# wkvong/multimodal-baby

Measured on AMD Instinct MI355X. Metric: image-text pairs/sec, CVCL ResNeXt+embed 224², bs256, 1/2/4/8 MI355X, higher is better.
Workload: dtype bf16; 1 GPU; C2 = BASELINE configs[1]: CVCL saycam_contrastive, frozen random-init ResNeXt-50 32x4d (BN train mode) + embedding mean-pool text encoder, E=512, L2-normalised, fixed tau 0.07, 224x224 frames + 3-word utterances; full step = fwd + InfoNCE + bwd(fc, embedding) + AdamW; per_gpu_batch=256, global_batch=256, negatives=local (single GPU), parallelism=dp1, trunk_streams=2

## Files before the change

### multimodal-baby_amd/csrc/gemm_pro.hip

```cpp
#include <cstdlib>

#include "cvcl_common.h"

namespace {

constexpr int PM = 64;
constexpr int PN = 256;

struct ProDev {
    const bf16_t* A; const bf16_t* W; bf16_t* C; const bf16_t* R;
    const float* a_scale; const float* a_shift; const float* c_scale; const float* c_shift; const float* r_scale; const float* r_shift;
    float* stats;
    int stats_acc;
    const float* centre;
    int M, N, lda, ldw, ldc, ldr;
    int tiles;
    const bf16_t* A2; const bf16_t* W2; const float* centre2;
    int lda2, ldw2;
};

enum { PRO_STATS = 0, PRO_STORE = 1, PRO_TAIL = 2, PRO_TAIL_DS = 3 };
constexpr int K2 = 64, KT2 = 2;
constexpr int X2BUF = PM * K2 * 2;

template <int KT> constexpr int pro_lds_bytes() { return 2 * PM * KT * 64 + 8 * 4096 + 6 * PN * 4 + 2 * 256 * 4 + 2 * X2BUF; }

template <int KT, int MODE, int D>
__global__ __launch_bounds__(512, 2) void gemm_pro_kernel(ProDev p) {
    constexpr bool TAIL = MODE == PRO_TAIL || MODE == PRO_TAIL_DS, DS = MODE == PRO_TAIL_DS;
    constexpr int K = KT * 32;
    constexpr int PITCH = K * 2;
    constexpr int CPR = K / 8;
    constexpr int NCH = PM * CPR / 512;
    constexpr int RPP = 512 / CPR;
    constexpr int ABUF = PM * PITCH;
    extern __shared__ __attribute__((aligned(16))) char smem[];
    const int tid = threadIdx.x, lane = tid & 63;
    const int wave = __builtin_amdgcn_readfirstlane(tid >> 6);
    const int wm = wave >> 2, wn = wave & 3;
    const int n0 = blockIdx.y * PN;

    bf16x8 fw[4][KT];
#pragma unroll
    for (int ni = 0; ni < 4; ++ni)
#pragma unroll
        for (int ks = 0; ks < KT; ++ks)
            fw[ni][ks] = *reinterpret_cast<const bf16x8*>(p.W + (long)(n0 + wn * 64 + ni * 16 + (lane & 15)) * p.ldw + ks * 32 + (lane >> 4) * 8);

    const int s_c = tid % CPR, s_r = tid / CPR;
    constexpr bool AFF_LDS = KT == 8;
    float* in_aff = reinterpret_cast<float*>(smem + 2 * ABUF + 8 * 4096 + 6 * PN * 4);
    char* x2buf = smem + 2 * ABUF + 8 * 4096 + 6 * PN * 4 + 2 * 256 * 4;
    const bool plain = p.a_scale == nullptr;
    const short fl = plain ? (short)-32768 : (short)0;
    const s16x2 floor2 = s16x2{fl, fl};
    f32x2 sc[4], sh[4];
#pragma unroll
    for (int e = 0; e < 4; ++e) { sc[e] = f32x2{1.f, 1.f}; sh[e] = f32x2{0.f, 0.f}; }
    if constexpr (AFF_LDS) {
        if (tid < K) { in_aff[tid] = plain ? 1.f : p.a_scale[tid]; in_aff[K + tid] = plain ? 0.f : p.a_shift[tid]; }
        __syncthreads();
    } else if (!plain) {
#pragma unroll
        for (int e = 0; e < 4; ++e) {
            sc[e] = f32x2{p.a_scale[s_c * 8 + 2 * e], p.a_scale[s_c * 8 + 2 * e + 1]};
            sh[e] = f32x2{p.a_shift[s_c * 8 + 2 * e], p.a_shift[s_c * 8 + 2 * e + 1]};
        }
    }
    u32x4 araw[D][NCH];
    auto load_a = [&](int tile, int slot) __attribute__((always_inline)) {
#pragma unroll
        for (int i = 0; i < NCH; ++i) {
            int m = tile * PM + s_r + RPP * i;
            if (m >= p.M) m = p.M - 1;
            araw[slot][i] = *reinterpret_cast<const u32x4*>(p.A + (long)m * p.lda + s_c * 8);
        }
    };
    auto stage_a = [&](int buf, int slot) __attribute__((always_inline)) {
        char* dst = smem + buf * ABUF;
        if constexpr (AFF_LDS) {
#pragma unroll
            for (int e = 0; e < 4; ++e) {
                sc[e] = *reinterpret_cast<const f32x2*>(in_aff + s_c * 8 + 2 * e);
                sh[e] = *reinterpret_cast<const f32x2*>(in_aff + K + s_c * 8 + 2 * e);
            }
        }
#pragma unroll
        for (int i = 0; i < NCH; ++i) {
            const int r = s_r + RPP * i;
            u32x4 v;
#pragma unroll
            for (int e = 0; e < 4; ++e) {
                const unsigned y = round2(__builtin_elementwise_fma(widen2(araw[slot][i][e]), sc[e], sh[e]));
                v[e] = __builtin_bit_cast(unsigned, __builtin_elementwise_max(__builtin_bit_cast(s16x2, y), floor2));
            }
            *reinterpret_cast<u32x4*>(dst + r * PITCH + ((s_c ^ (r & 15)) << 4)) = v;
        }
    };
    const int f_row = lane & 15, f_kc = lane >> 4;

    const int r_chunk = lane & 7, r_row0 = lane >> 3;
    float* aff = reinterpret_cast<float*>(smem + 2 * ABUF + 8 * 4096);
    if (tid < PN) aff[4 * PN + tid] = p.centre ? -p.centre[n0 + tid] : 0.f;
    if constexpr (DS) { if (tid < PN) aff[5 * PN + tid] = p.centre2 ? -p.centre2[n0 + tid] : 0.f; }
    const float* cen = aff + 4 * PN + wn * 64 + (lane >> 4) * 4;
    bf16x8 fw2[DS ? 4 : 1][DS ? KT2 : 1];
    u32x4 x2raw[DS ? D : 1];
    const int x_r = tid >> 3, x_c = tid & 7;
    if constexpr (DS) {
#pragma unroll
        for (int ni = 0; ni < 4; ++ni)
#pragma unroll
            for (int ks = 0; ks < KT2; ++ks)
                fw2[ni][ks] = *reinterpret_cast<const bf16x8*>(p.W2 + (long)(n0 + wn * 64 + ni * 16 + (lane & 15)) * p.ldw2 + ks * 32 + (lane >> 4) * 8);
    }
    auto load_x2 = [&](int tile, int slot) __attribute__((always_inline)) {
        int m = tile * PM + x_r;
        if (m >= p.M) m = p.M - 1;
        x2raw[slot] = *reinterpret_cast<const u32x4*>(p.A2 + (long)m * p.lda2 + x_c * 8);
    };
    auto stage_x2 = [&](int buf, int slot) __attribute__((always_inline)) {
        *reinterpret_cast<u32x4*>(x2buf + buf * X2BUF + x_r * 128 + ((x_c ^ (x_r & 7)) << 4)) = x2raw[slot];
    };
    if constexpr (TAIL) {
        if (tid < PN) {
            aff[tid] = p.c_scale[n0 + tid];
            aff[PN + tid] = p.c_shift[n0 + tid];
            aff[2 * PN + tid] = p.r_scale ? p.r_scale[n0 + tid] : 1.f;
            aff[3 * PN + tid] = p.r_scale ? p.r_shift[n0 + tid] : 0.f;
        }
    }
    bf16x8 rres[4];
    auto load_r = [&](int tile) __attribute__((always_inline)) {
#pragma unroll
        for (int j = 0; j < 4; ++j) {
            int m = tile * PM + wm * 32 + j * 8 + r_row0;
            if (m >= p.M) m = p.M - 1;
            rres[j] = *reinterpret_cast<const bf16x8*>(p.R + (long)m * p.ldr + n0 + wn * 64 + r_chunk * 8);
        }
    };
    f32x2 st_sum[8], st_sq[8];
#pragma unroll
    for (int e = 0; e < 8; ++e) { st_sum[e] = f32x2{0.f, 0.f}; st_sq[e] = f32x2{0.f, 0.f}; }

    char* stg = smem + 2 * ABUF + wave * 4096;
    const int e_row = lane & 15, e_wchunk = lane >> 5, e_wsub = ((lane >> 4) & 1) * 8;

    const int first = blockIdx.x;
    const int G = gridDim.x;
#pragma unroll
    for (int d = 0; d < D; ++d)
        if (first + d * G < p.tiles) {
            load_a(first + d * G, d);
            if constexpr (DS) load_x2(first + d * G, d);
        }
    if constexpr (MODE == PRO_TAIL) {
        if (first < p.tiles) load_r(first);
    }
    f32x4 acc[4][2];
    auto tile_stats = [&](int m0) __attribute__((always_inline)) {
#pragma unroll
        for (int mi = 0; mi < 2; ++mi) {
            const unsigned keep = m0 + mi * 16 + e_row < p.M ? 0xffffffffu : 0u;
#pragma unroll
            for (int ni = 0; ni < 4; ++ni)
#pragma unroll
                for (int h = 0; h < 2; ++h) {
                    const f32x2 f = widen2(round2(f32x2{acc[ni][mi][2 * h], acc[ni][mi][2 * h + 1]}) & keep);
                    st_sum[ni * 2 + h] += f;
                    st_sq[ni * 2 + h] = __builtin_elementwise_fma(f, f, st_sq[ni * 2 + h]);
                }
        }
    };
    int buf = 0;
    for (int tile = first; tile < p.tiles;) {
#pragma unroll
      for (int slot = 0; slot < D; ++slot) {
        if (tile >= p.tiles) break;
        stage_a(buf, slot);
        if constexpr (DS) stage_x2(buf, slot);
        __syncthreads();
        const int next = tile + G;
        if (tile + D * G < p.tiles) {
            load_a(tile + D * G, slot);
            if constexpr (DS) load_x2(tile + D * G, slot);
        }
        unsigned r2[DS ? 4 : 1][2][2];
        if constexpr (DS) {
            f32x4 acc2[4][2];
            const float* cen2 = aff + 5 * PN + wn * 64 + (lane >> 4) * 4;
#pragma unroll
            for (int ni = 0; ni < 4; ++ni) {
                const f32x4 c4 = *reinterpret_cast<const f32x4*>(cen2 + ni * 16);
#pragma unroll
                for (int mi = 0; mi < 2; ++mi) acc2[ni][mi] = c4;
            }
            const char* xb = x2buf + buf * X2BUF + (wm * 32 + f_row) * 128;
#pragma unroll
            for (int ks = 0; ks < KT2; ++ks) {
                bf16x8 fx[2];
#pragma unroll
                for (int mi = 0; mi < 2; ++mi)
                    fx[mi] = *reinterpret_cast<const bf16x8*>(xb + mi * 16 * 128 + (((ks * 4 + f_kc) ^ (f_row & 7)) << 4));
#pragma unroll
                for (int ni = 0; ni < 4; ++ni)
#pragma unroll
                    for (int mi = 0; mi < 2; ++mi)
                        acc2[ni][mi] = __builtin_amdgcn_mfma_f32_16x16x32_bf16(fw2[ni][ks], fx[mi], acc2[ni][mi], 0, 0, 0);
            }
#pragma unroll
            for (int ni = 0; ni < 4; ++ni)
#pragma unroll
                for (int mi = 0; mi < 2; ++mi) {
                    r2[ni][mi][0] = round2(f32x2{acc2[ni][mi][0], acc2[ni][mi][1]});
                    r2[ni][mi][1] = round2(f32x2{acc2[ni][mi][2], acc2[ni][mi][3]});
                }
        }
#pragma unroll
        for (int ni = 0; ni < 4; ++ni) {
            const f32x4 c4 = *reinterpret_cast<const f32x4*>(cen + ni * 16);
#pragma unroll
            for (int mi = 0; mi < 2; ++mi) acc[ni][mi] = c4;
        }
        const char* ab = smem + buf * ABUF + (wm * 32 + f_row) * PITCH;
#pragma unroll
        for (int ks = 0; ks < KT; ++ks) {
            bf16x8 fa[2];
#pragma unroll
            for (int mi = 0; mi < 2; ++mi)
                fa[mi] = *reinterpret_cast<const bf16x8*>(ab + mi * 16 * PITCH + (((ks * 4 + f_kc) ^ f_row) << 4));
#pragma unroll
            for (int ni = 0; ni < 4; ++ni)
#pragma unroll
                for (int mi = 0; mi < 2; ++mi)
                    acc[ni][mi] = __builtin_amdgcn_mfma_f32_16x16x32_bf16(fw[ni][ks], fa[mi], acc[ni][mi], 0, 0, 0);
        }
        const int m0 = tile * PM + wm * 32;
        if constexpr (MODE == PRO_STATS) {
            tile_stats(m0);
        } else if constexpr (DS) {
#pragma unroll
            for (int ni = 0; ni < 4; ++ni) {
                const float* t = aff + wn * 64 + ni * 16 + (lane >> 4) * 4;
                const f32x4 cs = *reinterpret_cast<const f32x4*>(t), cb = *reinterpret_cast<const f32x4*>(t + PN);
                const f32x4 rs = *reinterpret_cast<const f32x4*>(t + 2 * PN), rb = *reinterpret_cast<const f32x4*>(t + 3 * PN);
#pragma unroll
                for (int mi = 0; mi < 2; ++mi) {
                    bf16x4 q;
#pragma unroll
                    for (int e = 0; e < 4; ++e) {
                        const float y = fmaf((float)(bf16_t)acc[ni][mi][e], cs[e], cb[e]);
                        const float idv = fmaf(widen2(r2[ni][mi][e >> 1])[e & 1], rs[e], rb[e]);
                        q[e] = (bf16_t)fmaxf(y + idv, 0.f);
                    }
                    const int row = mi * 16 + e_row, chunk = ni * 2 + e_wchunk;
                    *reinterpret_cast<bf16x4*>(stg + row * 128 + ((chunk ^ ((row >> 1) & 7)) << 4) + e_wsub) = q;
                }
            }
#pragma unroll
            for (int j = 0; j < 4; ++j) {
                const int row = j * 8 + r_row0;
                const bf16x8 v = *reinterpret_cast<const bf16x8*>(stg + row * 128 + ((r_chunk ^ ((row >> 1) & 7)) << 4));
                const int m = m0 + row, n = n0 + wn * 64 + r_chunk * 8;
                if (m < p.M) stream_store(v, reinterpret_cast<bf16x8*>(p.C + (long)m * p.ldc + n));
            }
        } else {
#pragma unroll
            for (int mi = 0; mi < 2; ++mi)
#pragma unroll
                for (int ni = 0; ni < 4; ++ni) {
                    const bf16x4 q = {(bf16_t)acc[ni][mi][0], (bf16_t)acc[ni][mi][1], (bf16_t)acc[ni][mi][2], (bf16_t)acc[ni][mi][3]};
                    const int row = mi * 16 + e_row, chunk = ni * 2 + e_wchunk;
                    *reinterpret_cast<bf16x4*>(stg + row * 128 + ((chunk ^ ((row >> 1) & 7)) << 4) + e_wsub) = q;
                }
            float cs[8], cb[8], rs[8], rb[8];
            if constexpr (MODE == PRO_TAIL) {
                const float* t = aff + wn * 64 + r_chunk * 8;
#pragma unroll
                for (int e = 0; e < 8; ++e) { cs[e] = t[e]; cb[e] = t[PN + e]; rs[e] = t[2 * PN + e]; rb[e] = t[3 * PN + e]; }
            }
#pragma unroll
            for (int j = 0; j < 4; ++j) {
                const int row = j * 8 + r_row0;
                bf16x8 v = *reinterpret_cast<const bf16x8*>(stg + row * 128 + ((r_chunk ^ ((row >> 1) & 7)) << 4));
                const int m = m0 + row, n = n0 + wn * 64 + r_chunk * 8;
                if (m < p.M) {
                    if constexpr (MODE == PRO_TAIL) {
                        const bf16x8 r = rres[j];
#pragma unroll
                        for (int e = 0; e < 8; ++e) {
                            const float y = fmaf((float)v[e], cs[e], cb[e]);
                            const float idv = fmaf((float)r[e], rs[e], rb[e]);
                            v[e] = (bf16_t)fmaxf(y + idv, 0.f);
                        }
                    } else {
                        const u32x4 u = __builtin_bit_cast(u32x4, v);
#pragma unroll
                        for (int e = 0; e < 4; ++e) {
                            const f32x2 f = widen2(u[e]);
                            st_sum[e] += f;
                            st_sq[e] = __builtin_elementwise_fma(f, f, st_sq[e]);
                        }
                    }
                    stream_store(v, reinterpret_cast<bf16x8*>(p.C + (long)m * p.ldc + n));
                }
            }
            if constexpr (MODE == PRO_TAIL) {
                if (next < p.tiles) load_r(next);
            }
        }
        buf ^= 1;
        tile += G;
      }
    }

    if (!TAIL && p.stats) {
        __syncthreads();
        float* red = (float*)smem;
        if constexpr (MODE == PRO_STATS) {
#pragma unroll
            for (int e = 0; e < 8; ++e)
#pragma unroll
                for (int h = 0; h < 2; ++h)
#pragma unroll
                    for (int o = 1; o < 16; o <<= 1) {
                        st_sum[e][h] += __shfl_xor(st_sum[e][h], o, 64);
                        st_sq[e][h] += __shfl_xor(st_sq[e][h], o, 64);
                    }
            if ((lane & 15) == 0) {
#pragma unroll
                for (int ni = 0; ni < 4; ++ni)
#pragma unroll
                    for (int e = 0; e < 4; ++e) {
                        red[(wave * 2 + 0) * 64 + ni * 16 + (lane >> 4) * 4 + e] = st_sum[ni * 2 + (e >> 1)][e & 1];
                        red[(wave * 2 + 1) * 64 + ni * 16 + (lane >> 4) * 4 + e] = st_sq[ni * 2 + (e >> 1)][e & 1];
                    }
            }
        } else {
#pragma unroll
            for (int e = 0; e < 4; ++e)
#pragma unroll
                for (int h = 0; h < 2; ++h)
#pragma unroll
                    for (int o = 8; o <= 32; o <<= 1) {
                        st_sum[e][h] += __shfl_xor(st_sum[e][h], o, 64);
                        st_sq[e][h] += __shfl_xor(st_sq[e][h], o, 64);
                    }
            if (lane < 8) {
#pragma unroll
                for (int e = 0; e < 8; ++e) {
                    red[(wave * 2 + 0) * 64 + lane * 8 + e] = st_sum[e >> 1][e & 1];
                    red[(wave * 2 + 1) * 64 + lane * 8 + e] = st_sq[e >> 1][e & 1];
                }
            }
        }
        __syncthreads();
        if (tid < PN) {
            const int wn_ = tid >> 6, c = tid & 63, n = n0 + tid;
            cvcl_bn_stats_out(p.stats, p.stats_acc, blockIdx.x, p.N, n, red[(wn_ * 2 + 0) * 64 + c] + red[((wn_ + 4) * 2 + 0) * 64 + c],
                              red[(wn_ * 2 + 1) * 64 + c] + red[((wn_ + 4) * 2 + 1) * 64 + c]);
        }
    }
}

int pro_num_cus() {
    static int n = 0;
    if (!n) {
        int dev = 0;
        if (hipGetDevice(&dev) != hipSuccess || hipDeviceGetAttribute(&n, hipDeviceAttributeMultiprocessorCount, dev) != hipSuccess || n <= 0)
            n = 256;
    }
    return n;
}

template <int KT, int MODE, int D>
int pro_launch(const ProDev& d, dim3 grid, hipStream_t stream) {
    static CvclLdsAttr attr;
    constexpr int lds = pro_lds_bytes<KT>();
    if (const int rc = cvcl_raise_lds_limit(attr, (const void*)gemm_pro_kernel<KT, MODE, D>, lds, "cvcl_gemm_pro")) return rc;
    attr.mark();
    hipLaunchKernelGGL((gemm_pro_kernel<KT, MODE, D>), grid, dim3(512), lds, stream, d);
    CVCL_LAUNCH_CHECK();
    return CVCL_OK;
}

}

bool cvcl_gemm_pro_takes(const cvcl_gemm_args* a, bool stats) {
    const bool plain = !a->a_scale && !a->a_shift;
    if (!plain && (!a->a_scale || !a->a_shift || !a->a_relu)) return false;
    if (plain && (a->c_scale || a->A2 || a->W2)) return false;
    if ((a->K != 128 && a->K != 256) || a->N % PN != 0 || a->M < 1) return false;
    if (a->lda % 8 || a->ldw % 8 || (a->C && a->ldc % 8) || a->gather_stride > 1 || a->exp_scale || a->bias || a->C_pre || a->G) return false;
    if (!cvcl_aligned16(a->A) || !cvcl_aligned16(a->W) || !cvcl_aligned16(a->C) || !cvcl_aligned16(a->R)) return false;
    if (a->c_scale && a->A2)
        return a->c_shift && !a->R && a->C && !stats && a->act == CVCL_ACT_RELU && a->W2 && a->K2 == K2 && a->K == 128 && a->r_scale &&
               a->r_shift && a->lda2 % 8 == 0 && a->ldw2 % 8 == 0 && cvcl_aligned16(a->A2) && cvcl_aligned16(a->W2);
    if (a->A2 || a->W2) return false;
    if (a->c_scale) return a->c_shift && a->R && a->C && !stats && a->ldr % 8 == 0 && a->act == CVCL_ACT_RELU &&
                           (a->r_scale == nullptr) == (a->r_shift == nullptr);
    return !a->R && a->act == CVCL_ACT_NONE && (a->C || stats);
}
extern "C" int cvcl_gemm_pro_supported(const cvcl_gemm_args* a) { return a && cvcl_gemm_pro_takes(a, a->stats != nullptr); }

extern "C" int cvcl_gemm_pro_stats_rows(int M, int N) {
    const int tiles = cvcl_div_up(M, PM), ncol = N / PN;
    int g = pro_num_cus() / (ncol > 0 ? ncol : 1);
    if (g < 1) g = 1;
    return g > tiles ? tiles : g;
}

extern "C" int cvcl_gemm_pro(const cvcl_gemm_args* a, void* stream) {
    CVCL_CHECK_ARG(cvcl_gemm_pro_supported(a), "cvcl_gemm_pro: unsupported argument block");
    ProDev d;
    d.A = (const bf16_t*)a->A; d.W = (const bf16_t*)a->W; d.C = (bf16_t*)a->C; d.R = (const bf16_t*)a->R;
    d.a_scale = a->a_scale; d.a_shift = a->a_shift; d.c_scale = a->c_scale; d.c_shift = a->c_shift;
    d.r_scale = a->r_scale; d.r_shift = a->r_shift; d.stats = a->stats; d.centre = a->centre;
    d.stats_acc = a->stats && a->stats_rows == CVCL_STATS_ACCUMULATE;
    d.M = a->M; d.N = a->N; d.lda = a->lda; d.ldw = a->ldw; d.ldc = a->ldc; d.ldr = a->ldr;
    d.A2 = (const bf16_t*)a->A2; d.W2 = (const bf16_t*)a->W2; d.centre2 = a->centre2; d.lda2 = a->lda2; d.ldw2 = a->ldw2;
    d.tiles = cvcl_div_up(a->M, PM);
    const int gx = cvcl_gemm_pro_stats_rows(a->M, a->N);
    CVCL_CHECK_ARG(cvcl_stats_rows_fit(a, gx), "cvcl_gemm_pro: stats_rows %d < %d", a->stats_rows, gx);
    dim3 grid(gx, a->N / PN);
    const int mode = a->c_scale ? (a->A2 ? PRO_TAIL_DS : PRO_TAIL) : (a->C ? PRO_STORE : PRO_STATS);
    CvclProfScope prof(stream, CVCL_K_GEMM_PRO);
    hipStream_t st = (hipStream_t)stream;
    if (mode == PRO_TAIL_DS)
        return pro_launch<4, PRO_TAIL_DS, 2>(d, grid, st);
    if (a->K == 128) {
        if (mode == PRO_TAIL) return pro_launch<4, PRO_TAIL, 3>(d, grid, st);
        if (mode == PRO_STORE) return pro_launch<4, PRO_STORE, 3>(d, grid, st);
        return pro_launch<4, PRO_STATS, 3>(d, grid, st);
    }
    if (mode == PRO_TAIL) return pro_launch<8, PRO_TAIL, 2>(d, grid, st);
    if (mode == PRO_STORE) return pro_launch<8, PRO_STORE, 2>(d, grid, st);
    return pro_launch<8, PRO_STATS, 2>(d, grid, st);
}
```

Before: 52790 pairs/s.

## Add 32x512 wide-tile layout for K=256 N=512 tail GEMM with identity-residual path

For the PRO_TAIL mode with K=256 and N=512, a new wide tile layout is used. It has 32 rows by 512 columns, eight waves laid out 1x8 across N, and a persistent grid sized to the CU count, so one block covers the full N width and A rows are not re-read across column blocks. A second specialisation drops the residual scale/shift loads and FMA when r_scale is absent, which makes the residual an identity. The catch is that the smaller M tile holds more weight fragments per wave, which adds register pressure, and it may change occupancy.

```diff
diff --git a/multimodal-baby_amd/csrc/gemm_pro.hip b/multimodal-baby_amd/csrc/gemm_pro.hip
--- a/multimodal-baby_amd/csrc/gemm_pro.hip
+++ b/multimodal-baby_amd/csrc/gemm_pro.hip
@@ -6,6 +6,7 @@
 
 constexpr int PM = 64;
 constexpr int PN = 256;
+constexpr int WIDE_M = 32, WIDE_N = 512;
 
 struct ProDev {
     const bf16_t* A; const bf16_t* W; bf16_t* C; const bf16_t* R;
@@ -23,11 +24,17 @@
 constexpr int K2 = 64, KT2 = 2;
 constexpr int X2BUF = PM * K2 * 2;
 
-template <int KT> constexpr int pro_lds_bytes() { return 2 * PM * KT * 64 + 8 * 4096 + 6 * PN * 4 + 2 * 256 * 4 + 2 * X2BUF; }
-
-template <int KT, int MODE, int D>
+template <int KT, bool WIDE> constexpr int pro_lds_bytes() {
+    return WIDE ? 2 * WIDE_M * KT * 64 + 8 * 4096 + 6 * WIDE_N * 4 + 2 * 256 * 4
+                : 2 * PM * KT * 64 + 8 * 4096 + 6 * PN * 4 + 2 * 256 * 4 + 2 * X2BUF;
+}
+
+template <int KT, int MODE, int D, bool WIDE = false, bool RID = false>
 __global__ __launch_bounds__(512, 2) void gemm_pro_kernel(ProDev p) {
     constexpr bool TAIL = MODE == PRO_TAIL || MODE == PRO_TAIL_DS, DS = MODE == PRO_TAIL_DS;
+    static_assert(!WIDE || MODE == PRO_TAIL, "the 1 x 8 layout has the tail epilogue only");
+    static_assert(!RID || WIDE, "the identity-residual specialisation exists for the 1 x 8 layout only");
+    constexpr int PM = WIDE ? WIDE_M : 64, PN = WIDE ? WIDE_N : 256;
     constexpr int K = KT * 32;
     constexpr int PITCH = K * 2;
     constexpr int CPR = K / 8;
@@ -37,7 +44,7 @@
     extern __shared__ __attribute__((aligned(16))) char smem[];
     const int tid = threadIdx.x, lane = tid & 63;
     const int wave = __builtin_amdgcn_readfirstlane(tid >> 6);
-    const int wm = wave >> 2, wn = wave & 3;
+    const int wm = WIDE ? 0 : wave >> 2, wn = WIDE ? wave : wave & 3;
     const int n0 = blockIdx.y * PN;
 
     bf16x8 fw[4][KT];
@@ -126,8 +133,10 @@
         if (tid < PN) {
             aff[tid] = p.c_scale[n0 + tid];
             aff[PN + tid] = p.c_shift[n0 + tid];
-            aff[2 * PN + tid] = p.r_scale ? p.r_scale[n0 + tid] : 1.f;
-            aff[3 * PN + tid] = p.r_scale ? p.r_shift[n0 + tid] : 0.f;
+            if constexpr (!RID) {
+                aff[2 * PN + tid] = p.r_scale ? p.r_scale[n0 + tid] : 1.f;
+                aff[3 * PN + tid] = p.r_scale ? p.r_shift[n0 + tid] : 0.f;
+            }
         }
     }
     bf16x8 rres[4];
@@ -277,7 +286,10 @@
             if constexpr (MODE == PRO_TAIL) {
                 const float* t = aff + wn * 64 + r_chunk * 8;
 #pragma unroll
-                for (int e = 0; e < 8; ++e) { cs[e] = t[e]; cb[e] = t[PN + e]; rs[e] = t[2 * PN + e]; rb[e] = t[3 * PN + e]; }
+                for (int e = 0; e < 8; ++e) {
+                    cs[e] = t[e]; cb[e] = t[PN + e];
+                    if constexpr (!RID) { rs[e] = t[2 * PN + e]; rb[e] = t[3 * PN + e]; }
+                }
             }
 #pragma unroll
             for (int j = 0; j < 4; ++j) {
@@ -290,7 +302,8 @@
 #pragma unroll
                         for (int e = 0; e < 8; ++e) {
                             const float y = fmaf((float)v[e], cs[e], cb[e]);
-                            const float idv = fmaf((float)r[e], rs[e], rb[e]);
+                            float idv = (float)r[e];
+                            if constexpr (!RID) idv = fmaf(idv, rs[e], rb[e]);
                             v[e] = (bf16_t)fmaxf(y + idv, 0.f);
                         }
                     } else {
@@ -373,13 +386,13 @@
     return n;
 }
 
-template <int KT, int MODE, int D>
+template <int KT, int MODE, int D, bool WIDE = false, bool RID = false>
 int pro_launch(const ProDev& d, dim3 grid, hipStream_t stream) {
     static CvclLdsAttr attr;
-    constexpr int lds = pro_lds_bytes<KT>();
-    if (const int rc = cvcl_raise_lds_limit(attr, (const void*)gemm_pro_kernel<KT, MODE, D>, lds, "cvcl_gemm_pro")) return rc;
+    constexpr int lds = pro_lds_bytes<KT, WIDE>();
+    if (const int rc = cvcl_raise_lds_limit(attr, (const void*)gemm_pro_kernel<KT, MODE, D, WIDE, RID>, lds, "cvcl_gemm_pro")) return rc;
     attr.mark();
-    hipLaunchKernelGGL((gemm_pro_kernel<KT, MODE, D>), grid, dim3(512), lds, stream, d);
+    hipLaunchKernelGGL((gemm_pro_kernel<KT, MODE, D, WIDE, RID>), grid, dim3(512), lds, stream, d);
     CVCL_LAUNCH_CHECK();
     return CVCL_OK;
 }
@@ -428,6 +441,13 @@
     hipStream_t st = (hipStream_t)stream;
     if (mode == PRO_TAIL_DS)
         return pro_launch<4, PRO_TAIL_DS, 2>(d, grid, st);
+    if (mode == PRO_TAIL && a->K == 256 && a->N == WIDE_N) {
+        d.tiles = cvcl_div_up(a->M, WIDE_M);
+        const int cus = pro_num_cus();
+        const dim3 wide(cus < d.tiles ? cus : d.tiles, 1);
+        if (!a->r_scale) return pro_launch<8, PRO_TAIL, 2, true, true>(d, wide, st);
+        return pro_launch<8, PRO_TAIL, 2, true, false>(d, wide, st);
+    }
     if (a->K == 128) {
         if (mode == PRO_TAIL) return pro_launch<4, PRO_TAIL, 3>(d, grid, st);
         if (mode == PRO_STORE) return pro_launch<4, PRO_STORE, 3>(d, grid, st);
```

New measurement: 53280 pairs/s (median of 6 runs). About the same (+0.9%).
